# Disty0/sdnq

Hardware: AMD Instinct MI355X
Metric: quantized-matmul GOP/s (SDXL UNet int8 Linear step, bs=1) (higher is better)
Workload: dtype i8; 1 GPU; sdxl_int8: 741 quantized Linear layers of one denoising step, bs=1 (722 w8a8 GEMMs + 19 M=1 layers); parallelism=single GPU, launch=hipGraph replay, activations=bf16, distinct_activation_tensors=446, activation_quant_cache=True, requantized_weight_cache=True, fused_projections=False, linked_projection_groups=71, one_launch_linears=192, weights_dtype=int8, group_size=-1, use_quantized_matmul=True

## Files before the change

### sdnq_amd/csrc/gemm_aq.hip

```cpp
#include "gemm_dev.h"
#include "quant8_dev.h"

namespace {

constexpr int BK = 128, NW = 8, NT = NW * 64;

struct AqParams {
    const float* sb;
    const void* bias;
    void* out;
    int64_t ldc;
    int bias_dtype;
    const uint8_t* pf_ptr[4];
    int pf_lines[4];
    unsigned long long* trace;
#ifdef SDNQ_AQ_LAB
    int lab;
#endif
};

typedef unsigned short us2 __attribute__((ext_vector_type(2)));

template <int MM> struct AqMma;
template <> struct AqMma<SDNQ_MM_I8> {
    typedef v16i acc_t;
    typedef v4i frag_t;
    static constexpr int KB = 32;
    static __device__ __forceinline__ frag_t load(const uint8_t* s, int r, int ks, int fgrp) {
        return *(const v4i*)(s + r * 128 + (((ks * 2 + fgrp) ^ ((r >> 1) & 7)) << 4));
    }
    static __device__ __forceinline__ void mma(acc_t& c, const frag_t& w, const frag_t& x) { c = __builtin_amdgcn_mfma_i32_32x32x32_i8(w, x, c, 0, 0, 0); }
    static __device__ __forceinline__ float tof(const acc_t& c, int i) { return (float)c[i]; }
};
template <> struct AqMma<SDNQ_MM_FP8> {
    typedef v16f acc_t;
    typedef v8i frag_t;
    static constexpr int KB = 64;
    static __device__ __forceinline__ frag_t load(const uint8_t* s, int r, int ks, int fgrp) {
        const int sw = (r >> 1) & 7;
        const v4i lo = *(const v4i*)(s + r * 128 + (((ks * 4 + fgrp * 2) ^ sw) << 4));
        const v4i hi = *(const v4i*)(s + r * 128 + (((ks * 4 + fgrp * 2 + 1) ^ sw) << 4));
        return (v8i){lo[0], lo[1], lo[2], lo[3], hi[0], hi[1], hi[2], hi[3]};
    }
    static __device__ __forceinline__ void mma(acc_t& c, const frag_t& w, const frag_t& x) {
        c = __builtin_amdgcn_mfma_scale_f32_32x32x64_f8f6f4(w, x, c, 0, 0, 0, 0x7f7f7f7f, 0, 0x7f7f7f7f);
    }
    static __device__ __forceinline__ float tof(const acc_t& c, int i) { return c[i]; }
};

template <int X_T, int MM, bool HAS_BIAS, int NJ, int NSB, int BM, int BN>
__global__ __launch_bounds__(NT) void linear_aq_kernel(const uint16_t* __restrict__ x, const uint8_t* __restrict__ w, int ldx, int ldb, int M, int N,
                                                       int K, int tiles_m, int tiles_n, int group_m, AqParams p_) {
    SDNQ_KERNARGS_NOW("s"(x), "s"(w), "s"(ldx), "s"(ldb), "s"(M), "s"(N), "s"(K), "s"(tiles_m), "s"(tiles_n), "s"(group_m));
    const AqParams& p = p_;
    typedef AqMma<MM> MT;
    static_assert(BM % 32 == 0 && BN % 32 == 0 && (BM / 32) * (BN / 32) == NW, "one 32x32 accumulator per wave");
    constexpr int A_STAGE = BM * BK, B_STAGE = BN * BK;
    constexpr int PS = BM / (4 * NW);
    constexpr int PPW = BN / (8 * NW);
    static_assert(PS >= 1 && PS <= 2 && PS * 4 * NW == BM && PPW >= 1 && PPW * 8 * NW == BN && BN <= NT, "geometry");
    extern __shared__ __attribute__((aligned(1024))) uint8_t lds[];
    uint8_t* const ldsA = lds;
    uint8_t* const ldsB = lds + NJ * A_STAGE;
    float* const s_sb = (float*)(ldsB + NSB * B_STAGE);
    float* const s_bias = s_sb + BN;
    float* const s_xs = s_bias + BN;

    const int tid = threadIdx.x, lane = tid & 63;
    const int wave = __builtin_amdgcn_readfirstlane(tid >> 6);
    const int nwg = tiles_m * tiles_n;
    const int bid = blockIdx.x;
    if (bid >= nwg) {
        SDNQ_PREFETCH_LINES(tid, bid - nwg, NT, (int)gridDim.x - nwg, p);
        return;
    }
    const unsigned long long t_entry = __builtin_amdgcn_s_memtime();
    int tile_m, tile_n;
    grouped_tile(xcd_contiguous(bid, nwg), tiles_m, tiles_n, group_m, tile_m, tile_n);
    const int m0 = tile_m * BM, n0 = tile_n * BN;
    const int nk = K / BK;
    const int m_rows = (M - m0) < BM ? (M - m0) : BM, n_lim = (N - n0) < BN ? (N - n0) : BN;

    const auto rsX = SDNQ_MAKE_RSRC_N((const uint8_t*)x + (int64_t)m0 * ldx * 2, ((int64_t)(m_rows - 1) * ldx + K) * 2);
    v4i xr[PS][NJ];
    int qrow[PS];
#pragma unroll
    for (int ps = 0; ps < PS; ++ps) {
        qrow[ps] = wave * (4 * PS) + ps * 4 + (lane >> 4);
        const int rc = qrow[ps] < m_rows ? qrow[ps] : m_rows - 1;
        const int vo = rc * ldx * 2 + (lane & 15) * 16;
#pragma unroll
        for (int j = 0; j < NJ; ++j) xr[ps][j] = SDNQ_BUF_LOAD16(rsX, vo, j < nk ? j * 256 : 0x40000000);
    }
    const auto rsB = SDNQ_MAKE_RSRC_N(w + (int64_t)n0 * ldb, (int64_t)(n_lim - 1) * ldb + K);
    int voB[PPW];
#pragma unroll
    for (int u = 0; u < PPW; ++u) {
        const int r = (wave + u * NW) * 8 + (lane >> 3);
        const int rc = r < n_lim ? r : n_lim - 1;
        voB[u] = rc * ldb + (((lane & 7) ^ ((r >> 1) & 7)) << 4);
    }
    auto issueB = [&](int st, int slot) {
        const int s = st < nk ? st : 0;
#pragma unroll
        for (int u = 0; u < PPW; ++u) SDNQ_DMA16(rsB, ldsB + slot * B_STAGE + (wave + u * NW) * 1024, voB[u], s * BK);
    };
    constexpr int AHEAD = NSB - 1;
#pragma unroll
    for (int s = 0; s < AHEAD; ++s) issueB(s, s);
    __builtin_amdgcn_sched_barrier(0);
    SDNQ_KERNARGS_NOW("s"(p_.sb), "s"(p_.bias), "s"(p_.out), "s"(p_.ldc), "s"(p_.bias_dtype), "s"(p_.trace));
    if (p.trace != nullptr && tid == 0 && blockIdx.x < 1024) p.trace[blockIdx.x * 8] = t_entry;
    SDNQ_PHASE_STAMP(p.trace, 1);
    float ev_sb = 0.0f;
    u32 ev_bias = 0;
    if (tid < BN) {
        const int64_t gi = n0 + (tid < n_lim ? tid : n_lim - 1);
        ev_sb = p.sb[gi];
        if constexpr (HAS_BIAS) {
            if (p.bias_dtype == SDNQ_F32) ev_bias = ((const u32*)p.bias)[gi];
            else ev_bias = ((const uint16_t*)p.bias)[gi];
        }
    }

    constexpr float QMAX = (MM == SDNQ_MM_I8) ? 127.0f : 448.0f;
#pragma unroll
    for (int ps = 0; ps < PS; ++ps) {
        if (ps == 0) wait_vmcnt<(PS - 1) * NJ + PPW * AHEAD>();
        else wait_vmcnt<PPW * AHEAD>();
        us2 mx = {0, 0};
#pragma unroll
        for (int j = 0; j < NJ; ++j)
#pragma unroll
            for (int d = 0; d < 4; ++d)
                mx = __builtin_elementwise_max(mx, __builtin_bit_cast(us2, (u32)xr[ps][j][d] & 0x7fff7fffu));
        u32 m32 = __builtin_bit_cast(u32, mx);
#pragma unroll
        for (int s = 1; s <= 8; s <<= 1) {
            const u32 o = (u32)lane_xor_i32((int)m32, s);
            m32 = __builtin_bit_cast(u32, __builtin_elementwise_max(__builtin_bit_cast(us2, m32), __builtin_bit_cast(us2, o)));
        }
        u32 mb = (m32 & 0xffffu) > (m32 >> 16) ? (m32 & 0xffffu) : (m32 >> 16);
        constexpr u32 INF_BITS = X_T == SDNQ_BF16 ? 0x7f80u : 0x7c00u;
        if (__builtin_amdgcn_ballot_w64(mb > INF_BITS) != 0) {
            u32 mn = 0;
#pragma unroll
            for (int j = 0; j < NJ; ++j)
#pragma unroll
                for (int d = 0; d < 4; ++d) {
                    const u32 lo = (u32)xr[ps][j][d] & 0x7fffu, hi = ((u32)xr[ps][j][d] >> 16) & 0x7fffu;
                    mn = lo > INF_BITS ? mn : (lo > mn ? lo : mn);
                    mn = hi > INF_BITS ? mn : (hi > mn ? hi : mn);
                }
#pragma unroll
            for (int s = 1; s <= 8; s <<= 1) {
                const u32 o = (u32)lane_xor_i32((int)mn, s);
                mn = o > mn ? o : mn;
            }
            mb = mn;
        }
        const float amax = X_T == SDNQ_BF16 ? __uint_as_float(mb << 16) : f16_bits_to_f32((uint16_t)mb);
        const float scale = amax / QMAX;
        RowDiv rd;
        rd.set(scale);
        if ((lane & 15) == 0) s_xs[qrow[ps]] = scale;
        const int r = qrow[ps];
        uint8_t* dst = ldsA + r * 128 + ((lane & 1) << 3) + ((((lane & 15) >> 1) ^ ((r >> 1) & 7)) << 4);
        const bool all_fast = __builtin_amdgcn_ballot_w64(!rd.fast) == 0;
#ifdef SDNQ_AQ_LAB
        if (p.lab & 16) continue;
#endif
        if (all_fast) {
#pragma unroll
            for (int j = 0; j < NJ; ++j) {
                float v[8];
                const v4i t = xr[ps][j];
                Vec16<X_T>::unpack(make_uint4((u32)t[0], (u32)t[1], (u32)t[2], (u32)t[3]), v);
                const uint2 q = quant8_fast<MM>(v, rd);
                *(v2i*)(dst + j * A_STAGE) = (v2i){(int)q.x, (int)q.y};
            }
        } else {
#pragma unroll
            for (int j = 0; j < NJ; ++j) {
                float v[8];
                const v4i t = xr[ps][j];
                Vec16<X_T>::unpack(make_uint4((u32)t[0], (u32)t[1], (u32)t[2], (u32)t[3]), v);
                int isum = 0;
                const uint2 q = quant8<MM>(v, rd, isum);
                *(v2i*)(dst + j * A_STAGE) = (v2i){(int)q.x, (int)q.y};
            }
        }
    }
    if (tid < BN) {
        s_sb[tid] = ev_sb;
        if constexpr (HAS_BIAS)
            s_bias[tid] = p.bias_dtype == SDNQ_F32 ? __uint_as_float(ev_bias) : (p.bias_dtype == SDNQ_BF16 ? __uint_as_float(ev_bias << 16) : f16_bits_to_f32((uint16_t)ev_bias));
    }
    SDNQ_PHASE_STAMP(p.trace, 2);

    typename MT::acc_t acc;
#pragma unroll
    for (int e = 0; e < 16; ++e) acc[e] = 0;
    const int wm = wave / (BN / 32), wn = wave % (BN / 32);
    const int frow = lane & 31, fgrp = lane >> 5;
    constexpr int KS = BK / MT::KB;
    asm volatile("s_waitcnt lgkmcnt(0)" ::: "memory");
    typename MT::frag_t fa[2][KS], fb[2][KS];
    auto read_stage = [&](auto setc, auto ksc, int st, int slot) {
        constexpr int sx = decltype(setc)::value, ks = decltype(ksc)::value;
        fa[sx][ks] = MT::load(ldsA + (st < nk ? st : 0) * A_STAGE, wm * 32 + frow, ks, fgrp);
        fb[sx][ks] = MT::load(ldsB + slot * B_STAGE, wn * 32 + frow, ks, fgrp);
    };
    wait_vmcnt<(AHEAD - 1) * PPW>();
    __builtin_amdgcn_s_barrier();
    __builtin_amdgcn_sched_barrier(0);
    issueB(AHEAD, AHEAD);
    static_for_up<KS>([&](auto ksc) { read_stage(std::integral_constant<int, 0>{}, ksc, 0, 0); });
    int slot_c = 0;
#ifdef SDNQ_AQ_LAB
    const int lab = __builtin_amdgcn_readfirstlane(p.lab);
#else
    constexpr int lab = 0;
#endif
    auto half = [&](auto setc, int kt) {
        constexpr int sx = decltype(setc)::value;
        wait_vmcnt<(NSB - 2) * PPW>();
        asm volatile("s_waitcnt lgkmcnt(0)" ::: "memory");
        __builtin_amdgcn_sched_barrier(0);
        if (!(lab & 8)) __builtin_amdgcn_s_barrier();
        __builtin_amdgcn_sched_barrier(0);
        const int slot_free = slot_c;
        slot_c = (slot_c + 1 == NSB) ? 0 : slot_c + 1;
        static_for_up<KS>([&](auto ksc) {
            constexpr int ks = decltype(ksc)::value;
            if (!(lab & 4)) MT::mma(acc, fb[sx][ks], fa[sx][ks]);
            __builtin_amdgcn_sched_barrier(0);
            if (!(lab & 2)) read_stage(std::integral_constant<int, sx ^ 1>{}, ksc, kt + 1, slot_c);
            if constexpr (ks == 0) { if (!(lab & 1)) issueB(kt + NSB, slot_free); }
            __builtin_amdgcn_sched_barrier(0);
        });
    };
#pragma nounroll
    for (int kt = 0; kt < nk; kt += 2) {
        half(std::integral_constant<int, 0>{}, kt);
        if (kt + 1 < nk) half(std::integral_constant<int, 1>{}, kt + 1);
    }
    SDNQ_PHASE_STAMP(p.trace, 3);
    asm volatile("s_waitcnt vmcnt(0)" ::: "memory");
    __syncthreads();
    SDNQ_PHASE_STAMP(p.trace, 4);

    constexpr int OUT_ROW = BN * 2 + 16;
    static_assert(BM * OUT_ROW <= NJ * A_STAGE + NSB * B_STAGE, "output staging fits the operand area");
    {
        const int ml = wm * 32 + frow;
        const float sa = s_xs[ml];
#pragma unroll
        for (int q = 0; q < 4; ++q) {
            const int nl0 = wn * 32 + 8 * q + 4 * fgrp;
            float o[4];
#pragma unroll
            for (int e = 0; e < 4; ++e) {
                const float vv = MT::tof(acc, 4 * q + e) * sa;
                if constexpr (HAS_BIAS) o[e] = fmaf(vv, s_sb[nl0 + e], s_bias[nl0 + e]);
                else o[e] = vv * s_sb[nl0 + e];
            }
            *(uint2*)(lds + ml * OUT_ROW + nl0 * 2) = make_uint2(pack2<X_T>(o[0], o[1]), pack2<X_T>(o[2], o[3]));
        }
    }
    __syncthreads();
    SDNQ_PHASE_STAMP(p.trace, 5);
    constexpr int PPR = BN * 2 / 16;
#pragma unroll
    for (int v = tid; v < BM * PPR; v += NT) {
        const int r = v / PPR, c = v % PPR;
        if (r >= m_rows || c * 8 >= n_lim) continue;
        const uint4 val = *(const uint4*)(lds + r * OUT_ROW + c * 16);
        __builtin_nontemporal_store((v4i){(int)val.x, (int)val.y, (int)val.z, (int)val.w},
                                    (v4i*)((uint8_t*)p.out + ((int64_t)(m0 + r) * p.ldc + n0 + c * 8) * 2));
    }
    SDNQ_PHASE_STAMP(p.trace, 6);
}

std::atomic<unsigned long long*> g_aq_trace{nullptr};
std::atomic<int> g_aq_geometry{-1};

struct AqPlan { int geometry, bm, bn, tiles_m, tiles_n, group_m; int64_t prefetch_room; };
inline AqPlan aq_plan(int mm_dtype, int64_t m, int64_t n, int64_t k, int cus) {
    static const int geo_env = (int)env_int("SDNQ_HIP_FUSED_ROWQUANT_GEOMETRY", -1);
    static const int gm_env = (int)env_int("SDNQ_HIP_FUSED_ROWQUANT_GROUP_M", 8);
    int geo = g_aq_geometry.load(std::memory_order_relaxed);
    if (geo < 0) geo = geo_env;
    if (geo < 0) geo = (mm_dtype == SDNQ_MM_I8 && k > 640 && (n % 256) == 0 && ((m + 31) / 32) * (n / 256) <= cus) ? 1 : 0;
    AqPlan pl;
    pl.geometry = geo ? 1 : 0;
    pl.bm = geo ? 32 : 64;
    pl.bn = geo ? 256 : 128;
    pl.tiles_m = (int)((m + pl.bm - 1) / pl.bm);
    pl.tiles_n = (int)((n + pl.bn - 1) / pl.bn);
    const int gm = gm_env < 1 ? 1 : gm_env;
    pl.group_m = gm > pl.tiles_m ? pl.tiles_m : gm;
    pl.prefetch_room = (int64_t)cus - (int64_t)pl.tiles_m * pl.tiles_n;
    return pl;
}

template <int X_T, int MM, bool HAS_BIAS, int NJ, int NSB, int BM, int BN>
int launch_aq(const void* x, const void* w, int64_t ldx, int64_t m, int64_t n, int64_t k, const AqPlan& pl, AqParams p, hipStream_t s) {
    constexpr int LDS_BYTES = NJ * BM * BK + NSB * BN * BK + (2 * BN + BM) * 4;
    static_assert(LDS_BYTES <= 160 * 1024 && 2 * LDS_BYTES > 160 * 1024, "LDS budget: one workgroup per CU (aq_plan's prefetch room)");
    auto kern = linear_aq_kernel<X_T, MM, HAS_BIAS, NJ, NSB, BM, BN>;
    static std::atomic<uint64_t> attr_devices{0};
    if (LDS_BYTES > 64 * 1024 && !allow_dynamic_lds((const void*)kern, LDS_BYTES, attr_devices)) return SDNQ_ERR_LAUNCH;
    if (pl.bm != BM || pl.bn != BN) return SDNQ_ERR_LAUNCH;
    const int tiles_m = pl.tiles_m, tiles_n = pl.tiles_n, group_m = pl.group_m;
    const int64_t tiles = (int64_t)tiles_m * tiles_n;
    p.trace = g_aq_trace.load(std::memory_order_relaxed);
#ifdef SDNQ_AQ_LAB
    p.lab = (int)env_int("SDNQ_HIP_AQ_LAB", 0);
#endif
    const int pf_wgs = sdnq_internal_take_prefetch(pl.prefetch_room, NT, p.pf_ptr, p.pf_lines);
    hipLaunchKernelGGL(kern, dim3((unsigned)(tiles + pf_wgs)), dim3(NT), LDS_BYTES, s, (const uint16_t*)x, (const uint8_t*)w, (int)ldx, (int)k, (int)m,
                       (int)n, (int)k, tiles_m, tiles_n, group_m, p);
    SDNQ_CHECK_LAUNCH();
    return SDNQ_OK;
}

}

extern "C" int sdnq_hip_linear_w8a8_fused_supported(int mm_dtype, int x_dtype, int out_dtype, int64_t m, int64_t n, int64_t k) {
    static const int64_t on = env_int("SDNQ_HIP_FUSED_ROWQUANT", 1), max_tn = env_int("SDNQ_HIP_FUSED_ROWQUANT_MAX_TILES_N", 12),
                         min_m = env_int("SDNQ_HIP_FUSED_ROWQUANT_MIN_M", 33), min_k = env_int("SDNQ_HIP_FUSED_ROWQUANT_MIN_K", 128),
                         max_k = env_int("SDNQ_HIP_FUSED_ROWQUANT_MAX_K", 1280);
    static const int64_t fp8_on = env_int("SDNQ_HIP_FUSED_ROWQUANT_FP8", 0);
    if (!on) return 0;
    if (mm_dtype != SDNQ_MM_I8 && !(mm_dtype == SDNQ_MM_FP8 && fp8_on)) return 0;
    if ((x_dtype != SDNQ_BF16 && x_dtype != SDNQ_F16) || out_dtype != x_dtype) return 0;
    if (m < min_m || n <= 0 || (n % 8) != 0 || k <= 0 || (k % 128) != 0 || k > 1280) return 0;
    const int64_t tiles_m = (m + 63) / 64, tiles_n = (n + 127) / 128;
    if (tiles_n > max_tn || k < min_k || k > max_k) return 0;
    if (tiles_m * tiles_n > (int64_t)cu_count()) return 0;
    return 1;
}

extern "C" int sdnq_hip_linear_w8a8_fused(int mm_dtype, const void* x, int x_dtype, int64_t m, int64_t k, int64_t ldx, const void* b,
                                          const float* sb, const void* bias, int bias_dtype, void* out, int out_dtype, int64_t n,
                                          sdnq_stream_t stream) {
    if (!x || !b || !sb || !out) return SDNQ_ERR_NULL;
    if (mm_dtype != SDNQ_MM_I8 && mm_dtype != SDNQ_MM_FP8) return SDNQ_ERR_DTYPE;
    if ((x_dtype != SDNQ_BF16 && x_dtype != SDNQ_F16) || out_dtype != x_dtype) return SDNQ_ERR_UNSUPPORTED;
    if (bias && (bias_dtype < 0 || bias_dtype > 2)) return SDNQ_ERR_DTYPE;
    if (m <= 0 || n <= 0 || k <= 0 || ldx < k || (n % 8) != 0) return SDNQ_ERR_SHAPE;
    if ((k % 128) != 0 || k > 1280) return SDNQ_ERR_UNSUPPORTED;
    if (m > 0x7fffffffll / 2 || n > 0x7fffffffll || ldx * 2 * 64 > 0x7fffffffll || k * 128 > 0x7fffffffll) return SDNQ_ERR_SHAPE;
    if (((uintptr_t)x % 16) || ((uintptr_t)b % 16) || ((uintptr_t)out % 16) || ((ldx * 2) % 16)) return SDNQ_ERR_ALIGN;
    AqParams p{};
    p.sb = sb; p.bias = bias; p.out = out; p.ldc = n; p.bias_dtype = bias_dtype;
    hipStream_t s = (hipStream_t)stream;
    const AqPlan pl = aq_plan(mm_dtype, m, n, k, cu_count());
#define AQ_G(XT, MMV, HB, NJV) (pl.geometry ? launch_aq<XT, MMV, HB, NJV, 3, 32, 256>(x, b, ldx, m, n, k, pl, p, s) : launch_aq<XT, MMV, HB, NJV, 4, 64, 128>(x, b, ldx, m, n, k, pl, p, s))
#define AQ_NJ(XT, MMV, HB) (k <= 640 ? AQ_G(XT, MMV, HB, 5) : AQ_G(XT, MMV, HB, 10))
#define AQ_B(XT, MMV) (bias ? AQ_NJ(XT, MMV, true) : AQ_NJ(XT, MMV, false))
#define AQ_X(MMV) (x_dtype == SDNQ_BF16 ? AQ_B(SDNQ_BF16, MMV) : AQ_B(SDNQ_F16, MMV))
    return mm_dtype == SDNQ_MM_I8 ? AQ_X(SDNQ_MM_I8) : AQ_X(SDNQ_MM_FP8);
#undef AQ_X
#undef AQ_B
#undef AQ_NJ
#undef AQ_G
}

void sdnq_internal_aq_trace(unsigned long long* device_buf) { g_aq_trace.store(device_buf, std::memory_order_relaxed); }

void sdnq_internal_aq_geometry(int geometry) { g_aq_geometry.store(geometry < 0 ? -1 : (geometry ? 1 : 0), std::memory_order_relaxed); }

void sdnq_internal_aq_plan(int mm_dtype, long long m, long long n, long long k, int cus, long long* out) {
    const AqPlan pl = aq_plan(mm_dtype, m, n, k, cus);
    out[0] = pl.geometry; out[1] = pl.bm; out[2] = pl.bn; out[3] = pl.tiles_m; out[4] = pl.tiles_n; out[5] = pl.group_m; out[6] = pl.prefetch_room;
}
```

Measured before the change: 612,000 GOP/s.

## Extend fused row-quant GEMM to tall tiles and two-resident workgroups

```diff
diff --git a/sdnq_amd/csrc/gemm_aq.hip b/sdnq_amd/csrc/gemm_aq.hip
--- a/sdnq_amd/csrc/gemm_aq.hip
+++ b/sdnq_amd/csrc/gemm_aq.hip
@@ -54,11 +54,12 @@
     SDNQ_KERNARGS_NOW("s"(x), "s"(w), "s"(ldx), "s"(ldb), "s"(M), "s"(N), "s"(K), "s"(tiles_m), "s"(tiles_n), "s"(group_m));
     const AqParams& p = p_;
     typedef AqMma<MM> MT;
-    static_assert(BM % 32 == 0 && BN % 32 == 0 && (BM / 32) * (BN / 32) == NW, "one 32x32 accumulator per wave");
+    constexpr int NACC = (BM / 32) * (BN / 32) / NW;
+    static_assert(BM % 32 == 0 && BN % 32 == 0 && NACC * NW == (BM / 32) * (BN / 32) && NACC >= 1 && NACC <= 2, "one or two 32x32 accumulators per wave");
     constexpr int A_STAGE = BM * BK, B_STAGE = BN * BK;
     constexpr int PS = BM / (4 * NW);
     constexpr int PPW = BN / (8 * NW);
-    static_assert(PS >= 1 && PS <= 2 && PS * 4 * NW == BM && PPW >= 1 && PPW * 8 * NW == BN && BN <= NT, "geometry");
+    static_assert(PS >= 1 && PS <= 4 && PS * 4 * NW == BM && PPW >= 1 && PPW * 8 * NW == BN && BN <= NT, "geometry");
     extern __shared__ __attribute__((aligned(1024))) uint8_t lds[];
     uint8_t* const ldsA = lds;
     uint8_t* const ldsB = lds + NJ * A_STAGE;
@@ -126,8 +127,9 @@
     constexpr float QMAX = (MM == SDNQ_MM_I8) ? 127.0f : 448.0f;
 #pragma unroll
     for (int ps = 0; ps < PS; ++ps) {
-        if (ps == 0) wait_vmcnt<(PS - 1) * NJ + PPW * AHEAD>();
-        else wait_vmcnt<PPW * AHEAD>();
+        static_for_up<PS>([&](auto pc) {
+            if (decltype(pc)::value == ps) wait_vmcnt<(PS - 1 - decltype(pc)::value) * NJ + PPW * AHEAD>();
+        });
         us2 mx = {0, 0};
 #pragma unroll
         for (int j = 0; j < NJ; ++j)
@@ -198,17 +200,20 @@
     }
     SDNQ_PHASE_STAMP(p.trace, 2);
 
-    typename MT::acc_t acc;
-#pragma unroll
-    for (int e = 0; e < 16; ++e) acc[e] = 0;
-    const int wm = wave / (BN / 32), wn = wave % (BN / 32);
+    typename MT::acc_t acc[NACC];
+#pragma unroll
+    for (int a = 0; a < NACC; ++a)
+#pragma unroll
+        for (int e = 0; e < 16; ++e) acc[a][e] = 0;
+    const int wm = (wave / (BN / 32)) * NACC, wn = wave % (BN / 32);
     const int frow = lane & 31, fgrp = lane >> 5;
     constexpr int KS = BK / MT::KB;
     asm volatile("s_waitcnt lgkmcnt(0)" ::: "memory");
-    typename MT::frag_t fa[2][KS], fb[2][KS];
+    typename MT::frag_t fa[2][NACC][KS], fb[2][KS];
     auto read_stage = [&](auto setc, auto ksc, int st, int slot) {
         constexpr int sx = decltype(setc)::value, ks = decltype(ksc)::value;
-        fa[sx][ks] = MT::load(ldsA + (st < nk ? st : 0) * A_STAGE, wm * 32 + frow, ks, fgrp);
+#pragma unroll
+        for (int a = 0; a < NACC; ++a) fa[sx][a][ks] = MT::load(ldsA + (st < nk ? st : 0) * A_STAGE, (wm + a) * 32 + frow, ks, fgrp);
         fb[sx][ks] = MT::load(ldsB + slot * B_STAGE, wn * 32 + frow, ks, fgrp);
     };
     wait_vmcnt<(AHEAD - 1) * PPW>();
@@ -233,7 +238,10 @@
         slot_c = (slot_c + 1 == NSB) ? 0 : slot_c + 1;
         static_for_up<KS>([&](auto ksc) {
             constexpr int ks = decltype(ksc)::value;
-            if (!(lab & 4)) MT::mma(acc, fb[sx][ks], fa[sx][ks]);
+            if (!(lab & 4)) {
+#pragma unroll
+                for (int a = 0; a < NACC; ++a) MT::mma(acc[a], fb[sx][ks], fa[sx][a][ks]);
+            }
             __builtin_amdgcn_sched_barrier(0);
             if (!(lab & 2)) read_stage(std::integral_constant<int, sx ^ 1>{}, ksc, kt + 1, slot_c);
             if constexpr (ks == 0) { if (!(lab & 1)) issueB(kt + NSB, slot_free); }
@@ -252,8 +260,9 @@
 
     constexpr int OUT_ROW = BN * 2 + 16;
     static_assert(BM * OUT_ROW <= NJ * A_STAGE + NSB * B_STAGE, "output staging fits the operand area");
-    {
-        const int ml = wm * 32 + frow;
+#pragma unroll
+    for (int a = 0; a < NACC; ++a) {
+        const int ml = (wm + a) * 32 + frow;
         const float sa = s_xs[ml];
 #pragma unroll
         for (int q = 0; q < 4; ++q) {
@@ -261,7 +270,7 @@
             float o[4];
 #pragma unroll
             for (int e = 0; e < 4; ++e) {
-                const float vv = MT::tof(acc, 4 * q + e) * sa;
+                const float vv = MT::tof(acc[a], 4 * q + e) * sa;
                 if constexpr (HAS_BIAS) o[e] = fmaf(vv, s_sb[nl0 + e], s_bias[nl0 + e]);
                 else o[e] = vv * s_sb[nl0 + e];
             }
@@ -285,33 +294,48 @@
 std::atomic<unsigned long long*> g_aq_trace{nullptr};
 std::atomic<int> g_aq_geometry{-1};
 
-struct AqPlan { int geometry, bm, bn, tiles_m, tiles_n, group_m; int64_t prefetch_room; };
+constexpr int64_t AQ_TALL_MAX_K = 640;
+
+struct AqPlan { int geometry, bm, bn, tiles_m, tiles_n, group_m, resident; int64_t prefetch_room; };
 inline AqPlan aq_plan(int mm_dtype, int64_t m, int64_t n, int64_t k, int cus) {
     static const int geo_env = (int)env_int("SDNQ_HIP_FUSED_ROWQUANT_GEOMETRY", -1);
     static const int gm_env = (int)env_int("SDNQ_HIP_FUSED_ROWQUANT_GROUP_M", 8);
+    static const int gm_tall_env = (int)env_int("SDNQ_HIP_FUSED_ROWQUANT_GROUP_M_TALL", 8);
+    static const int tall = env_int("SDNQ_HIP_FUSED_ROWQUANT_TALL_GEOMETRY", 2) == 3 ? 3 : 2;
+    struct Geo { int bm, bn, resident; };
+    static constexpr Geo GEOS[4] = {{64, 128, 1}, {32, 256, 1}, {64, 128, 2}, {128, 128, 1}};
+    const bool tall_ok = mm_dtype == SDNQ_MM_I8 && k <= AQ_TALL_MAX_K;
+    auto tiles_of = [&](int g) { return ((m + GEOS[g].bm - 1) / GEOS[g].bm) * ((n + GEOS[g].bn - 1) / GEOS[g].bn); };
     int geo = g_aq_geometry.load(std::memory_order_relaxed);
     if (geo < 0) geo = geo_env;
-    if (geo < 0) geo = (mm_dtype == SDNQ_MM_I8 && k > 640 && (n % 256) == 0 && ((m + 31) / 32) * (n / 256) <= cus) ? 1 : 0;
+    if (geo > 3 || (geo >= 2 && !tall_ok)) geo = -1;
+    if (geo < 0) {
+        if (mm_dtype == SDNQ_MM_I8 && k > 640 && (n % 256) == 0 && ((m + 31) / 32) * (n / 256) <= cus) geo = 1;
+        else if (tall_ok && tiles_of(0) > cus && tiles_of(tall) <= (int64_t)GEOS[tall].resident * cus) geo = tall;
+        else geo = 0;
+    }
     AqPlan pl;
-    pl.geometry = geo ? 1 : 0;
-    pl.bm = geo ? 32 : 64;
-    pl.bn = geo ? 256 : 128;
+    pl.geometry = geo;
+    pl.bm = GEOS[geo].bm;
+    pl.bn = GEOS[geo].bn;
+    pl.resident = GEOS[geo].resident;
     pl.tiles_m = (int)((m + pl.bm - 1) / pl.bm);
     pl.tiles_n = (int)((n + pl.bn - 1) / pl.bn);
-    const int gm = gm_env < 1 ? 1 : gm_env;
+    const int gm_e = geo >= 2 ? gm_tall_env : gm_env;
+    const int gm = gm_e < 1 ? 1 : gm_e;
     pl.group_m = gm > pl.tiles_m ? pl.tiles_m : gm;
-    pl.prefetch_room = (int64_t)cus - (int64_t)pl.tiles_m * pl.tiles_n;
+    pl.prefetch_room = (int64_t)pl.resident * cus - (int64_t)pl.tiles_m * pl.tiles_n;
     return pl;
 }
 
-template <int X_T, int MM, bool HAS_BIAS, int NJ, int NSB, int BM, int BN>
+template <int X_T, int MM, bool HAS_BIAS, int NJ, int NSB, int BM, int BN, int RESIDENT = 1>
 int launch_aq(const void* x, const void* w, int64_t ldx, int64_t m, int64_t n, int64_t k, const AqPlan& pl, AqParams p, hipStream_t s) {
     constexpr int LDS_BYTES = NJ * BM * BK + NSB * BN * BK + (2 * BN + BM) * 4;
-    static_assert(LDS_BYTES <= 160 * 1024 && 2 * LDS_BYTES > 160 * 1024, "LDS budget: one workgroup per CU (aq_plan's prefetch room)");
+    static_assert(RESIDENT * LDS_BYTES <= 160 * 1024 && (RESIDENT + 1) * LDS_BYTES > 160 * 1024, "LDS budget: exactly RESIDENT workgroups per CU (aq_plan's prefetch room)");
     auto kern = linear_aq_kernel<X_T, MM, HAS_BIAS, NJ, NSB, BM, BN>;
     static std::atomic<uint64_t> attr_devices{0};
     if (LDS_BYTES > 64 * 1024 && !allow_dynamic_lds((const void*)kern, LDS_BYTES, attr_devices)) return SDNQ_ERR_LAUNCH;
-    if (pl.bm != BM || pl.bn != BN) return SDNQ_ERR_LAUNCH;
+    if (pl.bm != BM || pl.bn != BN || pl.resident != RESIDENT) return SDNQ_ERR_LAUNCH;
     const int tiles_m = pl.tiles_m, tiles_n = pl.tiles_n, group_m = pl.group_m;
     const int64_t tiles = (int64_t)tiles_m * tiles_n;
     p.trace = g_aq_trace.load(std::memory_order_relaxed);
@@ -338,7 +362,7 @@
     if (m < min_m || n <= 0 || (n % 8) != 0 || k <= 0 || (k % 128) != 0 || k > 1280) return 0;
     const int64_t tiles_m = (m + 63) / 64, tiles_n = (n + 127) / 128;
     if (tiles_n > max_tn || k < min_k || k > max_k) return 0;
-    if (tiles_m * tiles_n > (int64_t)cu_count()) return 0;
+    if (tiles_m * tiles_n > (int64_t)cu_count() && aq_plan(mm_dtype, m, n, k, cu_count()).geometry < 2) return 0;
     return 1;
 }
 
@@ -351,26 +375,34 @@
     if (bias && (bias_dtype < 0 || bias_dtype > 2)) return SDNQ_ERR_DTYPE;
     if (m <= 0 || n <= 0 || k <= 0 || ldx < k || (n % 8) != 0) return SDNQ_ERR_SHAPE;
     if ((k % 128) != 0 || k > 1280) return SDNQ_ERR_UNSUPPORTED;
-    if (m > 0x7fffffffll / 2 || n > 0x7fffffffll || ldx * 2 * 64 > 0x7fffffffll || k * 128 > 0x7fffffffll) return SDNQ_ERR_SHAPE;
+    if (m > 0x7fffffffll / 2 || n > 0x7fffffffll || ldx * 2 * 128 > 0x7fffffffll || k * 128 > 0x7fffffffll) return SDNQ_ERR_SHAPE;
     if (((uintptr_t)x % 16) || ((uintptr_t)b % 16) || ((uintptr_t)out % 16) || ((ldx * 2) % 16)) return SDNQ_ERR_ALIGN;
     AqParams p{};
     p.sb = sb; p.bias = bias; p.out = out; p.ldc = n; p.bias_dtype = bias_dtype;
     hipStream_t s = (hipStream_t)stream;
     const AqPlan pl = aq_plan(mm_dtype, m, n, k, cu_count());
-#define AQ_G(XT, MMV, HB, NJV) (pl.geometry ? launch_aq<XT, MMV, HB, NJV, 3, 32, 256>(x, b, ldx, m, n, k, pl, p, s) : launch_aq<XT, MMV, HB, NJV, 4, 64, 128>(x, b, ldx, m, n, k, pl, p, s))
+#define AQ_L(XT, MMV, HB, NJV, ...) launch_aq<XT, MMV, HB, NJV, __VA_ARGS__>(x, b, ldx, m, n, k, pl, p, s)
+#define AQ_G(XT, MMV, HB, NJV) (pl.geometry == 1 ? AQ_L(XT, MMV, HB, NJV, 3, 32, 256) : AQ_L(XT, MMV, HB, NJV, 4, 64, 128))
 #define AQ_NJ(XT, MMV, HB) (k <= 640 ? AQ_G(XT, MMV, HB, 5) : AQ_G(XT, MMV, HB, 10))
 #define AQ_B(XT, MMV) (bias ? AQ_NJ(XT, MMV, true) : AQ_NJ(XT, MMV, false))
 #define AQ_X(MMV) (x_dtype == SDNQ_BF16 ? AQ_B(SDNQ_BF16, MMV) : AQ_B(SDNQ_F16, MMV))
+#define AQ_TB(XT, ...) (bias ? AQ_L(XT, SDNQ_MM_I8, true, 5, __VA_ARGS__) : AQ_L(XT, SDNQ_MM_I8, false, 5, __VA_ARGS__))
+#define AQ_T(...) (x_dtype == SDNQ_BF16 ? AQ_TB(SDNQ_BF16, __VA_ARGS__) : AQ_TB(SDNQ_F16, __VA_ARGS__))
+    if (pl.geometry == 2) return AQ_T(2, 64, 128, 2);
+    if (pl.geometry == 3) return AQ_T(3, 128, 128, 1);
     return mm_dtype == SDNQ_MM_I8 ? AQ_X(SDNQ_MM_I8) : AQ_X(SDNQ_MM_FP8);
+#undef AQ_T
+#undef AQ_TB
 #undef AQ_X
 #undef AQ_B
 #undef AQ_NJ
 #undef AQ_G
+#undef AQ_L
 }
 
 void sdnq_internal_aq_trace(unsigned long long* device_buf) { g_aq_trace.store(device_buf, std::memory_order_relaxed); }
 
-void sdnq_internal_aq_geometry(int geometry) { g_aq_geometry.store(geometry < 0 ? -1 : (geometry ? 1 : 0), std::memory_order_relaxed); }
+void sdnq_internal_aq_geometry(int geometry) { g_aq_geometry.store(geometry < 0 ? -1 : (geometry <= 3 ? geometry : 1), std::memory_order_relaxed); }
 
 void sdnq_internal_aq_plan(int mm_dtype, long long m, long long n, long long k, int cus, long long* out) {
     const AqPlan pl = aq_plan(mm_dtype, m, n, k, cus);
```

Measured after the change: 619,900 GOP/s (median of 6 runs). 1.01x the previous value.
